# TJUMMG/OCPG

Hardware: AMD Instinct MI355X
Metric: clips/sec fwd+bwd (5x384x640, R101) (higher is better)
Workload: dtype bf16

## Files before the change

include/ocpg_hip.h:

```cpp
#ifndef OCPG_HIP_H
#define OCPG_HIP_H
#include <stdint.h>

#ifdef __cplusplus
extern "C" {
#endif

int ocpg_msda_fwd_f32(const float* value, const int64_t* shapes, const int64_t* level_start,
                      const float* loc, const float* attn,
                      int N, int S, int M, int D, int L, int Lq, int P,
                      float* out, const int64_t* shapes_host, void* stream);
int ocpg_msda_fwd_f64(const double* value, const int64_t* shapes, const int64_t* level_start,
                      const double* loc, const double* attn,
                      int N, int S, int M, int D, int L, int Lq, int P,
                      double* out, void* stream);

int ocpg_msda_bwd_f32(const float* value, const int64_t* shapes, const int64_t* level_start,
                      const float* loc, const float* attn, const float* grad_out,
                      int N, int S, int M, int D, int L, int Lq, int P,
                      float* grad_value, float* grad_loc, float* grad_attn,
                      const int64_t* shapes_host, void* stream);
int ocpg_msda_bwd_value_f32(const float* loc, const float* attn, const float* grad_out,
                            int N, int S, int M, int D, int L, int Lq, int P,
                            float* grad_value, const int64_t* shapes_host, void* stream);
// ... 37 lines not shown
                      int N, int S, int M, int D, int L, int Lq, int P,
                      float* grad_value, float* grad_loc, float* grad_attn,
                      const int64_t* shapes_host, int* sel_state, int dtype, void* stream);
int ocpg_msda_bwd_value_h16(const float* loc, const float* attn, const void* grad_out,
                            int N, int S, int M, int D, int L, int Lq, int P,
                            float* grad_value, const int64_t* shapes_host, int* sel_state, int dtype, void* stream);
int ocpg_msda_bwd_locattn_h16(const void* value, const int64_t* shapes, const int64_t* level_start,
                              const float* loc, const float* attn, const void* grad_out,
                              int N, int S, int M, int D, int L, int Lq, int P,
                              float* grad_loc, float* grad_attn, int dtype, void* stream);
int ocpg_msda_fused_fwd_h16(const void* value, const int64_t* shapes, const int64_t* level_start,
                            const float* qproj, const float* ref,
                            int N, int S, int M, int D, int L, int Lq, int P,
                            void* out, float* loc_out, float* attn_out, int dtype, void* stream);
int ocpg_msda_fused_bwd_qproj_h16(const void* value, const int64_t* shapes, const int64_t* level_start,
                                  const float* loc, const float* attn, const void* grad_out,
                                  int N, int S, int M, int D, int L, int Lq, int P,
                                  float* grad_qproj, int dtype, void* stream);

int ocpg_bn_act_fwd(const void* x, const float* scale, const float* shift, const void* skip, void* y,
                    long long n_outer, int C, long long inner, int relu, int dtype, void* stream);
int ocpg_bn_act_bwd(const void* gy, const void* y, const float* scale, void* gx, void* gskip,
                    long long n_outer, int C, long long inner, int relu, int dtype, void* stream);

int ocpg_gemm_dgrad_bn_tile(long long M, int N, int K);
int ocpg_gemm_dgrad_bn(const void* a, const void* w, const void* c, const void* mask, const float* scale, void* out, void* out_skip,
                       long long M, int N, int K, int dtype, int tile, void* stream);

int ocpg_gemm_dgrad_mask(const void* a, const void* w, const void* mask, float scale, void* out, float* colsum_part, long long M, int N,
                         int K, int dtype, int tile, void* stream);
int ocpg_gemm_bias_relu_dropout_fwd(const void* x, const void* w, const void* bias, float p, unsigned long long seed,
                                    unsigned long long offset, const unsigned long long* rng_base, void* h, long long M, int N, int K,
                                    int dtype, int tile, int round_gemm, void* stream);

int ocpg_win_attn_fwd(const void* qkv, const float* biasT, const int* region, float scale, int BW, int NW, int N, int H,
                      int head_dim, void* out, float* lse, int dtype, void* stream);
int ocpg_win_attn_bwd(const void* qkv, const float* bias, const float* biasT, const int* region, float scale, int BW, int NW,
                      int N, int H, int head_dim, const void* out, const void* dout, const float* lse, void* dqkv, float* Dbuf,
                      float* dbiasT, int dtype, void* stream);

int ocpg_win_attn_bwd_mfma(const void* qkv, const float* bias, const float* biasT, const int* region, float scale, int BW, int NW, int N,
                           int H, int head_dim, const void* out, const void* dout, const float* lse, void* dqkv, float* Dbuf, void* dS,
                           int dtype, void* stream);

int ocpg_win_attn_dtable_supported(int N, int head_dim, int dtype, int T);
int ocpg_win_attn_bwd_mfma_dtable(const void* qkv, const float* bias, const float* biasT, const int* region, float scale, int BW, int NW,
                                  int N, int H, int head_dim, const void* out, const void* dout, const float* lse, void* dqkv, float* Dbuf,
                                  const int* tok_code, int code_off, int T, float* partials, float* dtable, int dtype, void* stream);

int ocpg_dynmask_fwd_f32(const float* feats, const float* params, const float* refpix, int BT, int Q, int C, int H, int W,
                         int stride, float* out, float* pre1, void* stream);

int ocpg_dynmask_bwd_pre_f32(const float* dout, const float* pre1, const float* params, int BT, int Q, int C, int H, int W,
                             int stride, float* dpre, float* part, float* w0d, void* stream);
int ocpg_dynmask_bwd_fin_f32(const float* part, const float* params, const float* refpix, const float* dw0, int BT, int Q, int C,
                             int H, int W, float* dparams, float* dref, void* stream);

int ocpg_im2col3x3_nhwc(const void* x, int N, int H, int W, int C, int stride, int dil, void* cols, int dtype, void* stream);
int ocpg_col2im3x3_nhwc(const void* dcols, int N, int H, int W, int C, int stride, int dil, void* dx, int dtype, void* stream);

int ocpg_conv3x3_mfma_fwd(const void* x, const void* w, const float* scale, const float* bias, int relu, int N, int H, int W,
                          int Cin, int Cout, int stride, void* y, void* stream);
int ocpg_conv3x3_mfma_fwd_cols(const void* x, const void* w, const float* scale, const float* bias, int relu, int N, int H, int W, int Cin,
                               int Cout, int stride, void* y, void* cols, void* stream);
int ocpg_conv3x3_mfma_dgrad(const void* dy, const void* wT, int N, int H, int W, int Cin, int Cout, int stride, void* dx,
                            void* stream);
int ocpg_conv3x3_mfma_dgrad_masked(const void* dy, const void* wT, const void* mask_y, const float* scale, int N, int H, int W, int Cin,
                                   int Cout, int stride, void* dx, void* stream);
int ocpg_conv3x3_mfma_dgrad_w(const void* dy, const void* w, const void* mask_y, const float* scale, int N, int H, int W, int Cin, int Cout,
                              int stride, void* dx, void* stream);
int ocpg_conv3x3_mfma_body_splits(long long M, int ncols, int kchannels);
int ocpg_conv3x3_mfma_fwd_bn_splitk(const void* x, const void* w, const float* scale, const float* shift, int relu, int N, int H, int W, int Cin,
                                    int Cout, int stride, int splits, float* part, void* y, void* stream);
int ocpg_conv3x3_mfma_dgrad_w_splitk(const void* dy, const void* w, const void* mask_y, const float* scale, int N, int H, int W, int Cin,
                                     int Cout, int stride, int splits, float* part, void* dx, void* stream);
int ocpg_conv3x3_mfma_wgrad_splits(int N, int H, int W, int Cin, int Cout, int stride);
int ocpg_conv3x3_mfma_wgrad(const void* gz, const void* x, int N, int H, int W, int Cin, int Cout, int stride, void* part, void* stream);
int ocpg_conv3x3_mfma_fwd_cols_h16(const void* x, const void* w, const float* scale, const float* bias, int relu, int N, int H, int W, int Cin,
                                   int Cout, int stride, void* y, void* cols, int dtype, void* stream);
int ocpg_conv3x3_mfma_dgrad_w_h16(const void* dy, const void* w, const void* mask_y, const float* scale, int N, int H, int W, int Cin, int Cout,
                                  int stride, void* dx, int dtype, void* stream);
int ocpg_conv3x3_mfma_wgrad_h16(const void* gz, const void* x, int N, int H, int W, int Cin, int Cout, int stride, void* part, int dtype,
                                void* stream);
int ocpg_conv3x3_mfma_dgrad_w_s2(const void* dy, const void* w, const void* mask_y, const float* scale, int N, int H, int W, int Cin, int Cout,
                                 int stride, void* dx, void* stream);
int ocpg_conv3x3_mfma_dgrad_w_s2_h16(const void* dy, const void* w, const void* mask_y, const float* scale, int N, int H, int W, int Cin, int Cout,
                                     int stride, void* dx, int dtype, void* stream);

int ocpg_conv3x3_mfma_splits(int N, int H, int W, int Cin, int Cout, int stride);
int ocpg_conv3x3_mfma_fwd_splitk(const void* x, const void* w, const float* bias, int N, int H, int W, int Cin, int Cout, int stride,
                                 int splits, float* part, void* y, int out_dt, void* cols, void* stream);
int ocpg_conv3x3_mfma_fwd_splitk_h16(const void* x, const void* w, const float* bias, int N, int H, int W, int Cin, int Cout, int stride,
                                     int splits, float* part, void* y, int out_dt, void* cols, int dtype, void* stream);

int ocpg_gemm(const void* A, const void* B, void* C, const void* bias, int dtype, int out_dtype, int transA, int transB,
              long long M, long long N, long long K, long long lda, long long ldb, long long ldc, long long batch,
              long long strideA, long long strideB, long long strideC, float alpha, float beta, void* stream);
long long ocpg_gemm_plans(void);
long long ocpg_gemm_tuned(long long* changed);
long long ocpg_gemm_tune_rejected(void);
void ocpg_gemm_set_tuning(int on);
long long ocpg_gemm_export_picks(long long* buf, long long cap_pairs);
int ocpg_gemm_import_picks(const long long* buf, long long n_pairs);
int ocpg_gemm_bn_act(const void* A, const void* W, void* D, const float* scale, const float* shift, const void* skip, int relu, int dtype,
                     long long M, long long N, long long K, void* stream);

int ocpg_levelset_fwd_f32(const float* x, const float* feats, const float* box, int Lr, int N, int C, int CF, int h, int w, float* sums,
                          float* coef, float* loss, void* stream);
int ocpg_levelset_bwd_f32(const float* x, const float* feats, const float* box, const float* coef, const float* gloss, int Lr, int N,
                          int C, int CF, int h, int w, float* gx, float* gfeat, void* stream);
int ocpg_proj_fwd_f32(const float* x, const float* tcmax, const float* trmax, const float* tcmean, const float* trmean, int Lr, int B,
                      int T, int H, int W, float* colstat, float* rowstat, float* IU, float* loss, void* stream);
int ocpg_proj_bwd_f32(const float* x, const float* tcmax, const float* trmax, const float* tcmean, const float* trmean,
                      const float* colstat, const float* rowstat, const float* IU, const float* gloss, int Lr, int B, int T, int H, int W,
                      float* Gc, float* Gr, float* gx, void* stream);

int ocpg_matcher_cost_f32(const float* logits, const float* boxes, const float* masks, long long sl, long long sb, long long st,
                          long long sq, const float* gt, const float* tboxes, const float* valid, const long long* labels, int Lr,
                          int B, int T, int Q, int K, int h, int w, float wc, float wb, float wg, float wm, float wd, float* sums,
                          float* cost, int* bad, void* stream);

int ocpg_dropout_add_ln_fwd(const void* x, const float* res, const float* gamma, const float* beta, long long R, int C, float eps, float p,
                            unsigned long long seed, unsigned long long offset, const unsigned long long* rng_base, int x_dtype, float* y,
                            float* mean, float* rstd, void* stream);
int ocpg_dropout_add_ln_bwd(const float* gy, const void* x, const float* res, const float* gamma, const float* mean, const float* rstd,
                            long long R, int C, float p, unsigned long long seed, unsigned long long offset, const unsigned long long* rng_base,
                            int x_dtype, void* gx, float* gres, float* dgb_part, void* stream);
long long ocpg_dropout_add_ln_bwd_slots(long long R);
int ocpg_dropout_add_ln_fwd_ex(const void* x, const float* res, const float* gamma, const float* beta, long long R, int C, float eps, float p,
                               unsigned long long seed, unsigned long long offset, const unsigned long long* rng_base, int x_dtype, float* y,
                               float* mean, float* rstd, const float* addend, float* y_add, void* y_lp, int lp_dtype, void* stream);
int ocpg_dropout_add_ln_bwd_ex(const void* g0, int g0_dtype, const void* g1, int g1_dtype, const void* g2, int g2_dtype, const void* x,
                               const float* res, const float* gamma, const float* mean, const float* rstd, long long R, int C, float p,
                               unsigned long long seed, unsigned long long offset, const unsigned long long* rng_base, int x_dtype, void* gx,
                               float* gres, float* dgb_part, float* gxsum_part, void* stream);
int ocpg_bias_relu_dropout_fwd(const void* a, const void* bias, long long R, int C, float p, unsigned long long seed,
                               unsigned long long offset, const unsigned long long* rng_base, int dtype, void* h, void* stream);
int ocpg_bias_relu_dropout_bwd(const void* gh, const void* h, long long R, int C, float p, int dtype, void* ga, float* dbias_part,
                               void* stream);
long long ocpg_bias_relu_dropout_bwd_slots(long long R, int C, int dtype);

int ocpg_multi_cast(const long long* srcs, const long long* dsts, const long long* numels, const long long* chunk_prefix, int n,
                    long long total_chunks, int src_dtype, int dst_dtype, void* stream);
int ocpg_multi_cast_sum(const long long* srcs, const long long* dsts, const long long* numels, const long long* chunk_prefix,
                        const long long* splits, const long long* strides, int n, long long total_chunks, int src_dtype, int dst_dtype,
                        void* stream);
long long ocpg_colsum_blocks(long long R);
int ocpg_colsum_partials(const void* x, long long R, int C, int dtype, float* part, void* stream);

int ocpg_grad_norm_clip(const long long* grads, const long long* numels, const long long* chunk_prefix, int n, long long total_chunks,
                        float max_norm, float* partials, float* norm_and_coef, void* stream);
int ocpg_adamw_step(const long long* params, const long long* grads, const long long* exp_avg, const long long* exp_avg_sq,
                    const long long* numels, const long long* chunk_prefix, const float* lr, const float* weight_decay, int n,
                    long long total_chunks, const float* norm_and_coef, double beta1, double beta2, double eps, long long step, void* stream);
int ocpg_grad_norm_clip_amp(const long long* grads, const long long* numels, const long long* chunk_prefix, int n, long long total_chunks,
                            float max_norm, float* partials, const float* grad_scale, const float* found_inf, double beta1, double beta2,
                            float* amp_state, void* stream);
int ocpg_adamw_step_amp(const long long* params, const long long* grads, const long long* exp_avg, const long long* exp_avg_sq,
                        const long long* numels, const long long* chunk_prefix, const float* lr, const float* weight_decay, int n,
                        long long total_chunks, const float* amp_state, double beta1, double beta2, double eps, void* stream);

int ocpg_det_loss_fwd_f32(const float* logits, const float* boxes, const long long* src, const float* valid, const long long* labels,
                          const float* tboxes, const float* num_boxes, float alpha, int Lr, int B, int T, int Q, int K, float* loss, int* bad,
                          void* stream);
int ocpg_det_loss_bwd_f32(const float* logits, const float* boxes, const long long* src, const float* valid, const long long* labels,
                          const float* tboxes, const float* num_boxes, const float* gloss, float alpha, int Lr, int B, int T, int Q, int K,
// ... 158 lines not shown
```

ocpg_amd/_lib.py:

```python
import ctypes
import glob
import os
import re

import torch

_HERE = os.path.dirname(os.path.abspath(__file__))
LIB_PATH = os.environ.get("OCPG_HIP_LIB") or os.path.join(_HERE, "lib", "libocpg_hip.so")
_lib = None

DTYPE_CODE = {torch.float32: 0, torch.bfloat16: 1, torch.float16: 2}
H16_CODE = {torch.bfloat16: 1, torch.float16: 2}

_BY_VALUE = {"int": ctypes.c_int, "long long": ctypes.c_longlong, "unsigned long long": ctypes.c_ulonglong, "float": ctypes.c_float,
             "double": ctypes.c_double}
_RETURNS = {"int": ctypes.c_int, "long long": ctypes.c_longlong, "void": None, "const char*": ctypes.c_char_p}
_DECL = re.compile(r"([\w\s*]+?)\b(\w+)\s*\(([^()]*)\)")


def _declarations(text):
    text = re.sub(r"/\*.*?\*/", " ", text, flags=re.S)
    if "//" in text:
        raise ValueError("a // comment in the header: the signature parser reads block comments only")
    text = re.sub(r"^[ \t]*#.*$", "", text, flags=re.M)
    text = re.sub(r'extern\s+"C"\s*\{', "", text)
    text = re.sub(r"^[ \t]*\}[ \t]*$", "", text, flags=re.M)

    def norm(t):
        return re.sub(r"\s*\*\s*", "*", " ".join(t.split()))
    out = []
    for stmt in text.split(";"):
        if not stmt.strip():
            continue
        m = _DECL.fullmatch(stmt.strip())
        if m is None:
            raise ValueError(f"not a function declaration: {' '.join(stmt.split())!r}")
        params = []
        for p in m.group(3).split(","):
            if p.strip() in ("", "void"):
                continue
            t, pname = re.fullmatch(r"(.*?)(\w*)", p.strip(), flags=re.S).groups()
            params.append((norm(t), pname))
        out.append((norm(m.group(1)), m.group(2), params))
    return out


def parse_header(text):
    out = {}
    for ret, name, params in _declarations(text):
        if ret not in _RETURNS:
            raise ValueError(f"{name}: return type {ret!r} is not one of {sorted(_RETURNS)}")
        argtypes = []
        for t, pname in params:
            if "*" not in t and t not in _BY_VALUE:
                raise ValueError(f"{name}: parameter {pname!r} has by-value type {t!r}, not one of {sorted(_BY_VALUE)}")
            argtypes.append(ctypes.c_void_p if "*" in t else _BY_VALUE[t])
        out[name] = (_RETURNS[ret], argtypes)
    return out


_HEADERS = "".join(open(h).read() for h in sorted(glob.glob(os.path.join(os.path.dirname(_HERE), "include", "*.h"))))
_PARSED = parse_header(_HEADERS)
SIGNATURES = {name: argtypes for name, (_, argtypes) in _PARSED.items() if name != "ocpg_hip_version"}


_TIMING = {"on": False, "events": []}
_UNTIMED = frozenset(name for _, name, params in _declarations(_HEADERS)
                     if name in SIGNATURES and ("void*", "stream") not in params)


def enable_kernel_timing(on=True):
    _TIMING["on"] = on
    _TIMING["events"] = []


def collect_kernel_timing(work=None):
    torch.cuda.synchronize()
    out = {}
    for name, args, e0, e1 in _TIMING["events"]:
        d = out.setdefault(name, {"ms": 0.0, "n": 0, "work": 0.0, "modelled": 0})
        d["ms"] += e0.elapsed_time(e1)
        d["n"] += 1
        w = work(name, args) if work is not None else None
        if isinstance(w, tuple):
            d["work_lowp"] = d.get("work_lowp", 0.0) + (w[0] if w[1] else 0.0)
            w = w[0]
        if w is not None:
            d["work"] += w
            d["modelled"] += 1
    _TIMING["events"] = []
    _TIMING["on"] = False
    return out


CENSUS = {"on": False, "calls": {}}
CENSUS_ALSO = {"ocpg_conv3x3_mfma_dgrad_w_s2": "ocpg_conv3x3_mfma_dgrad_w", "ocpg_conv3x3_mfma_dgrad_w_s2_h16": "ocpg_conv3x3_mfma_dgrad_w_h16",
               "ocpg_dropout_add_ln_fwd_ex": "ocpg_dropout_add_ln_fwd", "ocpg_dropout_add_ln_bwd_ex": "ocpg_dropout_add_ln_bwd"}


def census(on=True):
    CENSUS["on"] = on
    if on:
        CENSUS["calls"] = {}
    return CENSUS["calls"]


class _Lib:

    def __init__(self, cdll):
        self._cdll = cdll

    def __getattr__(self, name):
        fn = getattr(self._cdll, name)
        if name not in SIGNATURES or name in _UNTIMED:
            setattr(self, name, fn)
            return fn
        timed = not name.startswith("ocpg_msda_")

        def call(*a):
            if CENSUS["on"]:
                rc = fn(*a)
                if rc == 0:
                    for k in (name, CENSUS_ALSO.get(name)):
                        if k is not None:
                            CENSUS["calls"][k] = CENSUS["calls"].get(k, 0) + 1
                return rc
            if not (timed and _TIMING["on"]):
                return fn(*a)
            e0, e1 = torch.cuda.Event(enable_timing=True), torch.cuda.Event(enable_timing=True)
            e0.record()
            rc = fn(*a)
            e1.record()
            _TIMING["events"].append((name, tuple(getattr(x, "value", x) for x in a), e0, e1))
            return rc
        setattr(self, name, call)
        return call


def lib():
    global _lib
    if _lib is None:
        if not os.path.exists(LIB_PATH):
            raise RuntimeError(
                f"{LIB_PATH} not found: build it with `python -m ocpg_amd.csrc.build` "
                "(hipcc --offload-arch=gfx950). The HIP extension is mandatory; there is no CPU/PyTorch fallback.")
        L = ctypes.CDLL(LIB_PATH)
        for name, (restype, argtypes) in _PARSED.items():
            fn = getattr(L, name)
            fn.argtypes = argtypes
            fn.restype = restype
        _lib = _Lib(L)
    return _lib


def check(status, what):
    if status != 0:
        if status <= -1000:
            raise RuntimeError(f"{what}: invalid argument #{-status - 1000}")
        raise RuntimeError(f"{what}: HIP error {-status}")


def stream_ptr():
    return ctypes.c_void_p(torch.cuda.current_stream().cuda_stream)


def require_gpu(name, t):
    if not t.is_cuda:
        raise RuntimeError(f"{name} must be a GPU tensor: Not implemented on the CPU")
    if not t.is_contiguous():
        raise RuntimeError(f"{name} tensor has to be contiguous")
```

ocpg_amd/csrc/conv3x3_wgrad.hip:

```cpp
#include <hip/hip_bf16.h>
#include <hip/hip_fp16.h>
#include <hip/hip_runtime.h>
#include <stdint.h>

#include <cstdlib>

#include "../../include/ocpg_hip.h"
#include "h16_elem.h"

namespace {

typedef ocpg_h16::h16x8 bf16x8;
typedef short s4 __attribute__((ext_vector_type(4)));
typedef ocpg_h16::f32x16 f32x16;
using ocpg_h16::Bf16;
using ocpg_h16::Fp16;

constexpr int NT = 256, TM = 64, TN = 64, LROW = 72;

__device__ __forceinline__ bf16x8 tr_frag(const short* tile, int r0, int pitch, int c0, int lane) {
  const int li = lane & 15, grp = lane >> 4, fh = lane >> 5;
  const short* p = tile + (r0 + (8 * fh + (li >> 2)) * pitch) * LROW + c0 + 16 * (grp & 1) + 4 * (li & 3);
  const s4 lo = __builtin_amdgcn_ds_read_tr16_b64_v4i16((__attribute__((address_space(3))) s4*)p);
  const s4 hi = __builtin_amdgcn_ds_read_tr16_b64_v4i16((__attribute__((address_space(3))) s4*)(p + 4 * pitch * LROW));
  bf16x8 r;
  r[0] = lo[0]; r[1] = lo[1]; r[2] = lo[2]; r[3] = lo[3]; r[4] = hi[0]; r[5] = hi[1]; r[6] = hi[2]; r[7] = hi[3];
  return r;
}

__device__ __forceinline__ uint4 keep(uint4 v, bool yes) { return make_uint4(yes ? v.x : 0u, yes ? v.y : 0u, yes ? v.z : 0u, yes ? v.w : 0u); }

struct WG {
  int N, H, W, Ho, Wo, Cin, Cout, stride, seg, xw, rows_per_split;
};

#define WGRAD_KERNEL conv3x3_wgrad
#define WGRAD_ELEM Bf16
#include "conv3x3_wgrad_kernel.h"
#undef WGRAD_KERNEL
#undef WGRAD_ELEM
#define WGRAD_KERNEL conv3x3_wgrad_f16
#define WGRAD_ELEM Fp16
#include "conv3x3_wgrad_kernel.h"
#undef WGRAD_KERNEL
#undef WGRAD_ELEM

inline int seg_of(int stride) { return stride == 1 ? 64 : 32; }

}

extern "C" {

int ocpg_conv3x3_mfma_wgrad_splits(int N, int H, int W, int Cin, int Cout, int stride) {
  if (N <= 0 || H <= 0 || W <= 0 || Cin <= 0 || Cout <= 0 || (stride != 1 && stride != 2)) return 0;
  const long long rows = (long long)N * ((H - 1) / stride + 1);
  const long long tiles = (long long)((Cout + TM - 1) / TM) * ((Cin + TN - 1) / TN);
  static const int target = [] { const char* e = std::getenv("OCPG_WGRAD_WGS"); return e && *e ? std::atoi(e) : 256; }();
  long long s = (target + tiles - 1) / tiles;
  if (s > rows) s = rows;
  if (s < 1) s = 1;
  const long long rps = (rows + s - 1) / s;
  return (int)((rows + rps - 1) / rps);
}

int ocpg_conv3x3_mfma_wgrad_h16(const void* gz, const void* x, int N, int H, int W, int Cin, int Cout, int stride, void* part, int dtype,
                                void* stream) {
  if (dtype != 1 && dtype != 2) return -1010;
  if (N < 0 || H <= 0 || W <= 0 || Cin <= 0 || Cout <= 0) return -1003;
  if ((stride != 1 && stride != 2) || Cin % 8 != 0 || Cout % 8 != 0) return -2000;
  if (N == 0) return 0;
  if (!gz) return -1001;
  if (!x) return -1002;
  if (!part) return -1009;
  WG g;
  g.N = N; g.H = H; g.W = W; g.Ho = (H - 1) / stride + 1; g.Wo = (W - 1) / stride + 1; g.Cin = Cin; g.Cout = Cout; g.stride = stride;
  g.seg = seg_of(stride);
  g.xw = (g.seg - 1) * stride + 3;
  const int splits = ocpg_conv3x3_mfma_wgrad_splits(N, H, W, Cin, Cout, stride);
  const long long rows = (long long)N * g.Ho;
  g.rows_per_split = (int)((rows + splits - 1) / splits);
  const dim3 grid((unsigned)((Cout + TM - 1) / TM), (unsigned)((Cin + TN - 1) / TN), (unsigned)splits);
  if (dtype == 2) {
    if (stride == 1) conv3x3_wgrad_f16<1, 64><<<grid, NT, 0, (hipStream_t)stream>>>((const __half*)gz, (const __half*)x, g, (__half*)part);
    else conv3x3_wgrad_f16<2, 32><<<grid, NT, 0, (hipStream_t)stream>>>((const __half*)gz, (const __half*)x, g, (__half*)part);
  } else if (stride == 1) {
    conv3x3_wgrad<1, 64><<<grid, NT, 0, (hipStream_t)stream>>>((const __hip_bfloat16*)gz, (const __hip_bfloat16*)x, g, (__hip_bfloat16*)part);
  } else {
    conv3x3_wgrad<2, 32><<<grid, NT, 0, (hipStream_t)stream>>>((const __hip_bfloat16*)gz, (const __hip_bfloat16*)x, g, (__hip_bfloat16*)part);
  }
  const hipError_t e = hipGetLastError();
  return e == hipSuccess ? 0 : -(int)e;
}

int ocpg_conv3x3_mfma_wgrad(const void* gz, const void* x, int N, int H, int W, int Cin, int Cout, int stride, void* part, void* stream) {
  return ocpg_conv3x3_mfma_wgrad_h16(gz, x, N, H, W, Cin, Cout, stride, part, 1, stream);
}

}
```

ocpg_amd/models/ops/functions/conv_bn_func.py:

```python
import os

import torch
from torch.autograd import Function
from torch.autograd.function import once_differentiable

from ...._lib import DTYPE_CODE as _DT, H16_CODE, check, lib

_H16 = H16_CODE.keys()
_CL = torch.channels_last
EPILOGUE = os.environ.get("OCPG_GEMM_EPILOGUE", "1") != "0"
FWD_COLS = os.environ.get("OCPG_CONV3X3_FWD_COLS", "0") != "0"
SKIP_GRAD_IN_GEMM = os.environ.get("OCPG_SKIP_GRAD_IN_GEMM", "1") != "0"
_SKIP_TOKENS = {}
PREMASK = os.environ.get("OCPG_PREMASK_DGRAD", "1") != "0"
_PREMASK_TOKENS = {}
FUSED_DGRAD_BN = os.environ.get("OCPG_FUSED_DGRAD_BN", "1") != "0"
_DGRAD_BN_DECLINED = (-2000, -2001, -2002)


def reset_skip_tokens():
    _SKIP_TOKENS.clear()
    _PREMASK_TOKENS.clear()


# ... 221 lines not shown
    return x.shape[1] >= 256 and (x.shape[1] * x.element_size()) % 16 == 0 and rows <= 12288


class Conv3x3BNAct(Function):
    @staticmethod
    def forward(ctx, x, w, scale, shift, relu, stride, dil, splits):
        n, c, h, wd = x.shape
        co = w.shape[0]
        ho, wo = (h - 1) // stride + 1, (wd - 1) // stride + 1
        m = n * ho * wo
        dt = _DT[x.dtype]
        L = lib()
        st = torch.cuda.current_stream().cuda_stream
        cols = torch.empty((m, 9 * c), dtype=x.dtype, device=x.device)
        check(L.ocpg_im2col3x3_nhwc(x.data_ptr(), n, h, wd, c, stride, dil, cols.data_ptr(), dt, st), "ocpg_im2col3x3_nhwc")
        w2 = w.permute(0, 2, 3, 1).reshape(co, 9 * c)
        if not w2.is_contiguous():
            w2 = w2.contiguous()
        y = torch.empty((n, co, ho, wo), dtype=x.dtype, device=x.device, memory_format=_CL)
        rc = L.ocpg_gemm_bn_act(cols.data_ptr(), w2.data_ptr(), y.data_ptr(), scale.data_ptr(), shift.data_ptr(), None, int(relu), dt, m, co,
                                9 * c, st) if EPILOGUE else -1105
        if rc and rc != -1105:
            check(rc, "ocpg_gemm_bn_act")
        if rc:
            check(L.ocpg_gemm(cols.data_ptr(), w2.data_ptr(), y.data_ptr(), None, dt, dt, 0, 1, m, co, 9 * c, 9 * c, 9 * c, co, 1, 0, 0, 0, 1.0,
                              0.0, st), "ocpg_gemm")
            check(L.ocpg_bn_act_fwd(y.data_ptr(), scale.data_ptr(), shift.data_ptr(), None, y.data_ptr(), m, co, 1, int(relu), dt, st),
                  "ocpg_bn_act_fwd")
        ctx.save_for_backward(cols, w2, y, scale)
        ctx.meta = (bool(relu), splits, (n, c, h, wd, ho, wo, stride, dil), w.shape)
        return y

    @staticmethod
    @once_differentiable
    def backward(ctx, gy):
        cols, w2, y, scale = ctx.saved_tensors
        relu, splits, (n, c, h, wd, ho, wo, stride, dil), wshape = ctx.meta
        co = w2.shape[0]
        m, k = cols.shape
        dt = _DT[y.dtype]
        L = lib()
        st = torch.cuda.current_stream().cuda_stream
        if gy.dtype != y.dtype or not gy.is_contiguous(memory_format=_CL):
            gy = gy.to(y.dtype).contiguous(memory_format=_CL)
        gz = torch.empty_like(y)
        check(L.ocpg_bn_act_bwd(gy.data_ptr(), y.data_ptr(), scale.data_ptr(), gz.data_ptr(), None, m, co, 1, int(relu), dt, st), "ocpg_bn_act_bwd")
        gx = gw = None
        if ctx.needs_input_grad[0]:
            dcols = torch.empty((m, k), dtype=y.dtype, device=y.device)
            check(L.ocpg_gemm(gz.data_ptr(), w2.data_ptr(), dcols.data_ptr(), None, dt, dt, 0, 0, m, k, co, co, k, k, 1, 0, 0, 0, 1.0, 0.0, st),
                  "ocpg_gemm")
            gx = torch.empty((n, c, h, wd), dtype=y.dtype, device=y.device, memory_format=_CL)
            check(L.ocpg_col2im3x3_nhwc(dcols.data_ptr(), n, h, wd, c, stride, dil, gx.data_ptr(), dt, st), "ocpg_col2im3x3_nhwc")
        if ctx.needs_input_grad[1]:
            if splits > 1 and m % splits == 0:
                r = m // splits
                part = torch.empty((splits, co, k), dtype=y.dtype, device=y.device)
                check(L.ocpg_gemm(gz.data_ptr(), cols.data_ptr(), part.data_ptr(), None, dt, dt, 1, 0, co, k, r, co, k, k, splits, r * co, r * k,
                                  co * k, 1.0, 0.0, st), "ocpg_gemm")
                g2 = part.sum(0)
            else:
                g2 = torch.empty((co, k), dtype=y.dtype, device=y.device)
                check(L.ocpg_gemm(gz.data_ptr(), cols.data_ptr(), g2.data_ptr(), None, dt, dt, 1, 0, co, k, m, co, k, k, 1, 0, 0, 0, 1.0, 0.0, st),
                      "ocpg_gemm")
            gw = g2.view(co, 3, 3, c).permute(0, 3, 1, 2)
        return gx, gw, None, None, None, None, None, None


def conv3x3_bn_act(x, w, scale, shift, relu, stride, dil, splits):
    return Conv3x3BNAct.apply(x, w, scale, shift, relu, int(stride), int(dil), splits)


def eligible3x3_mfma(x, conv):
    if x.dtype == torch.float16 and (BODY_SPLITK or not DGRAD_OWN_WEIGHT):
        return False
    return (x.is_cuda and x.dim() == 4 and x.dtype in _H16 and conv.kernel_size == (3, 3) and conv.groups == 1
            and conv.bias is None and conv.stride[0] == conv.stride[1] and conv.stride[0] in (1, 2) and conv.dilation == (1, 1)
            and conv.padding == (1, 1) and conv.padding_mode == "zeros" and x.is_contiguous(memory_format=_CL)
            and x.shape[1] % 64 == 0 and conv.out_channels % 64 == 0 and x.shape[1] >= _MFMA_MIN_C and conv.out_channels >= _MFMA_MIN_C)


BODY_SPLITK = os.environ.get("OCPG_CONV3X3_SPLITK", "0") != "0"
WGRAD_OWN = os.environ.get("OCPG_WGRAD_OWN", "1") != "0"
DGRAD_OWN_WEIGHT = os.environ.get("OCPG_DGRAD_OWN_WEIGHT", "1") != "0"
DGRAD_S2_CLASSES = os.environ.get("OCPG_DGRAD_S2_CLASSES", "1") != "0"
_MFMA_MIN_C = int(os.environ.get("OCPG_MFMA_CONV3X3_MIN_C", "128"))


class Conv3x3MfmaBNAct(Function):

    @staticmethod
    def forward(ctx, x, w, scale, shift, relu, stride, splits):
        n, c, h, wd = x.shape
        co = w.shape[0]
        ho, wo = (h - 1) // stride + 1, (wd - 1) // stride + 1
        if not _both16(x, w):
            raise RuntimeError(f"Conv3x3MfmaBNAct: x and w must share one 16-bit dtype, got {x.dtype} and {w.dtype}")
        fp16 = x.dtype == torch.float16
        if fp16 and (BODY_SPLITK or not DGRAD_OWN_WEIGHT):
            raise RuntimeError("Conv3x3MfmaBNAct: OCPG_CONV3X3_SPLITK / OCPG_DGRAD_OWN_WEIGHT=0 select kernels that have no fp16 form")
        w2 = w.permute(0, 2, 3, 1)
        if not w2.is_contiguous():
            w2 = w2.contiguous()
        y = torch.empty((n, co, ho, wo), dtype=x.dtype, device=x.device, memory_format=_CL)
        st = torch.cuda.current_stream().cuda_stream
        cols = torch.empty((n * ho * wo, 9 * c), dtype=x.dtype, device=x.device) if (FWD_COLS and ctx.needs_input_grad[1]) else None
        sp = int(lib().ocpg_conv3x3_mfma_body_splits(n * ho * wo, co, c)) if (BODY_SPLITK and cols is None) else 1
        if sp > 1:
            part = torch.empty((sp, n * ho * wo, co), dtype=torch.float32, device=x.device)
            check(lib().ocpg_conv3x3_mfma_fwd_bn_splitk(x.data_ptr(), w2.data_ptr(), scale.data_ptr(), shift.data_ptr(), int(relu), n, h, wd, c, co, stride,
                                                        sp, part.data_ptr(), y.data_ptr(), st), "ocpg_conv3x3_mfma_fwd_bn_splitk")
        elif fp16:
            check(lib().ocpg_conv3x3_mfma_fwd_cols_h16(x.data_ptr(), w2.data_ptr(), scale.data_ptr(), shift.data_ptr(), int(relu), n, h, wd, c, co,
                                                       stride, y.data_ptr(), None if cols is None else cols.data_ptr(), 2, st),
                  "ocpg_conv3x3_mfma_fwd_cols_h16")
        else:
            check(lib().ocpg_conv3x3_mfma_fwd_cols(x.data_ptr(), w2.data_ptr(), scale.data_ptr(), shift.data_ptr(), int(relu), n, h, wd, c, co, stride,
                                                   y.data_ptr(), None if cols is None else cols.data_ptr(), st), "ocpg_conv3x3_mfma_fwd_cols")
        ctx.has_cols = cols is not None
        if cols is not None:
            ctx.save_for_backward(x, w2, y, scale, cols)
        else:
            ctx.save_for_backward(x, w2, y, scale)
        from ...amp_cache import is_cast_copy
        ctx.meta = (bool(relu), splits, stride)
        ctx.w_cast = is_cast_copy(w)
        tok = _claim_token(x) if PREMASK else None
        ctx.premask = tok if (tok is not None and not tok["skip"] and ctx.needs_input_grad[0]) else None
        ctx.offer = (_offer_token(y, scale, False, "OCPG_FUSED_DGRAD_BN")
                     if (FUSED_DGRAD_BN and relu and any(ctx.needs_input_grad)) else None)
        return y

    @staticmethod
    @once_differentiable
    def backward(ctx, gy):
        x, w2, y, scale = ctx.saved_tensors[:4]
        relu, splits, stride = ctx.meta
        n, c, h, wd = x.shape
        co, ho, wo = y.shape[1], y.shape[2], y.shape[3]
        m, k = n * ho * wo, 9 * c
        dt = _DT[y.dtype]
        fp16 = dt == 2
        L = lib()
        st = torch.cuda.current_stream().cuda_stream
        if gy.dtype != y.dtype or not gy.is_contiguous(memory_format=_CL):
            gy = gy.to(y.dtype).contiguous(memory_format=_CL)
        fused = _take_token(ctx.offer, gy)
        if fused is not None:
            gz = gy
        else:
            gz = torch.empty_like(y)
            check(L.ocpg_bn_act_bwd(gy.data_ptr(), y.data_ptr(), scale.data_ptr(), gz.data_ptr(), None, m, co, 1, int(relu), dt, st), "ocpg_bn_act_bwd")
        gx = gw = None
        if ctx.needs_input_grad[0]:
            gx = torch.empty((n, c, h, wd), dtype=y.dtype, device=y.device, memory_format=_CL)
            tok = ctx.premask
            mask_ptr, scale_ptr = (x.data_ptr(), tok["scale"].data_ptr()) if tok is not None else (None, None)
            sp = int(L.ocpg_conv3x3_mfma_body_splits(n * h * wd, c, co)) if (BODY_SPLITK and DGRAD_OWN_WEIGHT and c % 8 == 0 and not fp16) else 1
            s2 = stride == 2 and DGRAD_S2_CLASSES
            if fp16:
                fn = L.ocpg_conv3x3_mfma_dgrad_w_s2_h16 if s2 else L.ocpg_conv3x3_mfma_dgrad_w_h16
                check(fn(gz.data_ptr(), w2.data_ptr(), mask_ptr, scale_ptr, n, h, wd, c, co, stride, gx.data_ptr(), 2, st),
                      "ocpg_conv3x3_mfma_dgrad_w_s2_h16" if s2 else "ocpg_conv3x3_mfma_dgrad_w_h16")
            elif sp > 1:
                part = torch.empty((sp, n * h * wd, c), dtype=torch.float32, device=y.device)
                check(L.ocpg_conv3x3_mfma_dgrad_w_splitk(gz.data_ptr(), w2.data_ptr(), mask_ptr, scale_ptr, n, h, wd, c, co, stride, sp, part.data_ptr(),
                                                         gx.data_ptr(), st), "ocpg_conv3x3_mfma_dgrad_w_splitk")
            elif DGRAD_OWN_WEIGHT and c % 8 == 0:
                fn = L.ocpg_conv3x3_mfma_dgrad_w_s2 if s2 else L.ocpg_conv3x3_mfma_dgrad_w
                check(fn(gz.data_ptr(), w2.data_ptr(), mask_ptr, scale_ptr, n, h, wd, c, co, stride, gx.data_ptr(), st),
                      "ocpg_conv3x3_mfma_dgrad_w_s2" if s2 else "ocpg_conv3x3_mfma_dgrad_w")
            else:
                wt = w2.permute(3, 1, 2, 0).contiguous()
                check(L.ocpg_conv3x3_mfma_dgrad_masked(gz.data_ptr(), wt.data_ptr(), mask_ptr, scale_ptr, n, h, wd, c, co, stride, gx.data_ptr(), st),
                      "ocpg_conv3x3_mfma_dgrad_masked")
            if tok is not None:
                _fill_token(tok, gx)
        if ctx.needs_input_grad[1]:
            from ...amp_cache import side_wgrad
            with side_wgrad(ctx.w_cast, gz, x) as sw:
                st = torch.cuda.current_stream().cuda_stream
                if WGRAD_OWN and not ctx.has_cols and c % 8 == 0 and co % 8 == 0:
                    sp = int(L.ocpg_conv3x3_mfma_wgrad_splits(n, h, wd, c, co, stride))
                    part = torch.empty((sp, co, k), dtype=y.dtype, device=y.device)
                    if fp16:
                        check(L.ocpg_conv3x3_mfma_wgrad_h16(gz.data_ptr(), x.data_ptr(), n, h, wd, c, co, stride, part.data_ptr(), 2, st),
                              "ocpg_conv3x3_mfma_wgrad_h16")
                    else:
                        check(L.ocpg_conv3x3_mfma_wgrad(gz.data_ptr(), x.data_ptr(), n, h, wd, c, co, stride, part.data_ptr(), st), "ocpg_conv3x3_mfma_wgrad")
                    g2 = _reduce_partials(part, ctx.w_cast) if sp > 1 else part[0]
                else:
                    if ctx.has_cols:
                        cols = ctx.saved_tensors[4]
                    else:
                        cols = torch.empty((m, k), dtype=y.dtype, device=y.device)
                        check(L.ocpg_im2col3x3_nhwc(x.data_ptr(), n, h, wd, c, stride, 1, cols.data_ptr(), dt, st), "ocpg_im2col3x3_nhwc")
                    if splits > 1 and m % splits == 0:
                        r = m // splits
                        part = torch.empty((splits, co, k), dtype=y.dtype, device=y.device)
                        check(L.ocpg_gemm(gz.data_ptr(), cols.data_ptr(), part.data_ptr(), None, dt, dt, 1, 0, co, k, r, co, k, k, splits, r * co, r * k,
                                          co * k, 1.0, 0.0, st), "ocpg_gemm")
                        g2 = _reduce_partials(part, ctx.w_cast)
                    else:
                        g2 = torch.empty((co, k), dtype=y.dtype, device=y.device)
                        check(L.ocpg_gemm(gz.data_ptr(), cols.data_ptr(), g2.data_ptr(), None, dt, dt, 1, 0, co, k, m, co, k, k, 1, 0, 0, 0, 1.0, 0.0, st),
                              "ocpg_gemm")
                gw = sw.publish(g2).view(co, 3, 3, c).permute(0, 3, 1, 2)
        return gx, gw, None, None, None, None, None


def conv3x3_mfma_bn_act(x, w, scale, shift, relu, stride, splits):
    return Conv3x3MfmaBNAct.apply(x, w, scale, shift, relu, int(stride), splits)


def eligible3x3_splitk(x, conv):
    if not (x.is_cuda and x.dim() == 4 and x.dtype in _H16 and conv.kernel_size == (3, 3) and conv.groups == 1
            and conv.stride[0] == conv.stride[1] and conv.stride[0] in (1, 2) and conv.dilation == (1, 1) and conv.padding == (1, 1)
            and conv.padding_mode == "zeros" and x.is_contiguous(memory_format=_CL) and x.shape[1] % 64 == 0 and conv.out_channels % 64 == 0):
        return False
    n, c, h, w = x.shape
    return int(lib().ocpg_conv3x3_mfma_splits(n, h, w, c, conv.out_channels, conv.stride[0])) > 1


class Conv3x3SplitK(Function):

    @staticmethod
    def forward(ctx, x, w, b, stride):
        n, c, h, wd = x.shape
        co = w.shape[0]
        ho, wo = (h - 1) // stride + 1, (wd - 1) // stride + 1
        m = n * ho * wo
        L = lib()
        st = torch.cuda.current_stream().cuda_stream
        w2 = w.permute(0, 2, 3, 1)
        if not w2.is_contiguous():
            w2 = w2.contiguous()
        if not _both16(x, w):
            raise RuntimeError(f"Conv3x3SplitK: x and w must share one 16-bit dtype, got {x.dtype} and {w.dtype}")
        splits = int(L.ocpg_conv3x3_mfma_splits(n, h, wd, c, co, stride))
        part = torch.empty((splits, m, co), dtype=torch.float32, device=x.device)
        y = torch.empty((n, co, ho, wo), dtype=x.dtype, device=x.device, memory_format=_CL)
        need_w = ctx.needs_input_grad[1]
        cols = torch.empty((m, 9 * c), dtype=x.dtype, device=x.device) if need_w else None
        bf = None if b is None else b.float()
        if x.dtype == torch.float16:
            check(L.ocpg_conv3x3_mfma_fwd_splitk_h16(x.data_ptr(), w2.data_ptr(), None if bf is None else bf.data_ptr(), n, h, wd, c, co, stride, splits,
                                                     part.data_ptr(), y.data_ptr(), 2, None if cols is None else cols.data_ptr(), 2, st),
                  "ocpg_conv3x3_mfma_fwd_splitk_h16")
        else:
            check(L.ocpg_conv3x3_mfma_fwd_splitk(x.data_ptr(), w2.data_ptr(), None if bf is None else bf.data_ptr(), n, h, wd, c, co, stride, splits,
                                                 part.data_ptr(), y.data_ptr(), 1, None if cols is None else cols.data_ptr(), st),
                  "ocpg_conv3x3_mfma_fwd_splitk")
        ctx.save_for_backward(w2, cols if need_w else w2)
        ctx.meta = (n, c, h, wd, ho, wo, stride, b is not None, need_w)
        return y

    @staticmethod
    @once_differentiable
    def backward(ctx, gy):
        w2, cols = ctx.saved_tensors
        n, c, h, wd, ho, wo, stride, has_b, need_w = ctx.meta
        co = w2.shape[0]
        m, k = n * ho * wo, 9 * c
        L = lib()
        st = torch.cuda.current_stream().cuda_stream
        dt = _DT[w2.dtype]
        if gy.dtype != w2.dtype or not gy.is_contiguous(memory_format=_CL):
            gy = gy.to(w2.dtype).contiguous(memory_format=_CL)
# ... 23 lines not shown
```

Measured before the change: 68.03.

## Add ring-buffered 3x3 conv weight-gradient kernel reusing input rows across output rows

Adds a new wgrad kernel that streams output-gradient rows through double-buffered LDS and keeps a ring of input rows. Each loaded input row is reused by all three vertical taps instead of being re-read per row. Global loads are prefetched several steps ahead in registers, and the 9 taps are split between two wave groups running at different priorities. It is enabled by default for eligible shapes and falls back to the old kernel when shapes are rejected, at the cost of higher register and LDS use and a more complex indexing scheme.

```diff
diff --git a/include/ocpg_hip.h b/include/ocpg_hip.h
--- a/include/ocpg_hip.h
+++ b/include/ocpg_hip.h
@@ -143,6 +143,9 @@
                                   int stride, void* dx, int dtype, void* stream);
 int ocpg_conv3x3_mfma_wgrad_h16(const void* gz, const void* x, int N, int H, int W, int Cin, int Cout, int stride, void* part, int dtype,
                                 void* stream);
+int ocpg_conv3x3_mfma_wgrad_ring(const void* gz, const void* x, int N, int H, int W, int Cin, int Cout, int stride, void* part, void* stream);
+int ocpg_conv3x3_mfma_wgrad_ring_h16(const void* gz, const void* x, int N, int H, int W, int Cin, int Cout, int stride, void* part, int dtype,
+                                     void* stream);
 int ocpg_conv3x3_mfma_dgrad_w_s2(const void* dy, const void* w, const void* mask_y, const float* scale, int N, int H, int W, int Cin, int Cout,
                                  int stride, void* dx, void* stream);
 int ocpg_conv3x3_mfma_dgrad_w_s2_h16(const void* dy, const void* w, const void* mask_y, const float* scale, int N, int H, int W, int Cin, int Cout,
diff --git a/ocpg_amd/_lib.py b/ocpg_amd/_lib.py
--- a/ocpg_amd/_lib.py
+++ b/ocpg_amd/_lib.py
@@ -95,6 +95,7 @@
 
 CENSUS = {"on": False, "calls": {}}
 CENSUS_ALSO = {"ocpg_conv3x3_mfma_dgrad_w_s2": "ocpg_conv3x3_mfma_dgrad_w", "ocpg_conv3x3_mfma_dgrad_w_s2_h16": "ocpg_conv3x3_mfma_dgrad_w_h16",
+               "ocpg_conv3x3_mfma_wgrad_ring": "ocpg_conv3x3_mfma_wgrad", "ocpg_conv3x3_mfma_wgrad_ring_h16": "ocpg_conv3x3_mfma_wgrad_h16",
                "ocpg_dropout_add_ln_fwd_ex": "ocpg_dropout_add_ln_fwd", "ocpg_dropout_add_ln_bwd_ex": "ocpg_dropout_add_ln_bwd"}
 
 
diff --git a/ocpg_amd/csrc/conv3x3_wgrad.hip b/ocpg_amd/csrc/conv3x3_wgrad.hip
--- a/ocpg_amd/csrc/conv3x3_wgrad.hip
+++ b/ocpg_amd/csrc/conv3x3_wgrad.hip
@@ -46,6 +46,21 @@
 #undef WGRAD_ELEM
 
 inline int seg_of(int stride) { return stride == 1 ? 64 : 32; }
+
+constexpr int NTR = 512;
+template <int V>
+struct IC { static constexpr int value = V; };
+
+#define WGRAD_RING_KERNEL conv3x3_wgrad_ring
+#define WGRAD_ELEM Bf16
+#include "conv3x3_wgrad_ring_kernel.h"
+#undef WGRAD_RING_KERNEL
+#undef WGRAD_ELEM
+#define WGRAD_RING_KERNEL conv3x3_wgrad_ring_f16
+#define WGRAD_ELEM Fp16
+#include "conv3x3_wgrad_ring_kernel.h"
+#undef WGRAD_RING_KERNEL
+#undef WGRAD_ELEM
 
 }
 
@@ -96,4 +111,42 @@
   return ocpg_conv3x3_mfma_wgrad_h16(gz, x, N, H, W, Cin, Cout, stride, part, 1, stream);
 }
 
+int ocpg_conv3x3_mfma_wgrad_ring_h16(const void* gz, const void* x, int N, int H, int W, int Cin, int Cout, int stride, void* part, int dtype,
+                                     void* stream) {
+  if (dtype != 1 && dtype != 2) return -1010;
+  if (N < 0 || H <= 0 || W <= 0 || Cin <= 0 || Cout <= 0) return -1003;
+  if ((stride != 1 && stride != 2) || Cin % 8 != 0 || Cout % 8 != 0) return -2000;
+  if ((W - 1) / stride + 1 > seg_of(stride)) return -2000;
+  if ((long long)W * Cin > 0x7fffffffLL || (long long)W * Cout > 0x7fffffffLL) return -2000;
+  if (N == 0) return 0;
+  if (!gz) return -1001;
+  if (!x) return -1002;
+  if (!part) return -1009;
+  WG g;
+  g.N = N; g.H = H; g.W = W; g.Ho = (H - 1) / stride + 1; g.Wo = (W - 1) / stride + 1; g.Cin = Cin; g.Cout = Cout; g.stride = stride;
+  g.seg = seg_of(stride);
+  g.xw = (g.seg - 1) * stride + 3;
+  const int splits = ocpg_conv3x3_mfma_wgrad_splits(N, H, W, Cin, Cout, stride);
+  const long long rows = (long long)N * g.Ho;
+  g.rows_per_split = (int)((rows + splits - 1) / splits);
+  const dim3 grid((unsigned)((Cout + TM - 1) / TM), (unsigned)((Cin + TN - 1) / TN), (unsigned)splits);
+  const hipStream_t st = (hipStream_t)stream;
+  const int ks = (g.Wo + 15) / 16;
+#define RING(S_, SEG_, KS_)                                                                                                  \
+  if (dtype == 2) conv3x3_wgrad_ring_f16<S_, SEG_, KS_><<<grid, NTR, 0, st>>>((const __half*)gz, (const __half*)x, g, (__half*)part); \
+  else conv3x3_wgrad_ring<S_, SEG_, KS_><<<grid, NTR, 0, st>>>((const __hip_bfloat16*)gz, (const __hip_bfloat16*)x, g, (__hip_bfloat16*)part)
+  if (stride == 1) {
+    if (ks == 1) { RING(1, 64, 1); } else if (ks == 2) { RING(1, 64, 2); } else if (ks == 3) { RING(1, 64, 3); } else { RING(1, 64, 4); }
+  } else {
+    if (ks == 1) { RING(2, 32, 1); } else { RING(2, 32, 2); }
+  }
+#undef RING
+  const hipError_t e = hipGetLastError();
+  return e == hipSuccess ? 0 : -(int)e;
 }
+
+int ocpg_conv3x3_mfma_wgrad_ring(const void* gz, const void* x, int N, int H, int W, int Cin, int Cout, int stride, void* part, void* stream) {
+  return ocpg_conv3x3_mfma_wgrad_ring_h16(gz, x, N, H, W, Cin, Cout, stride, part, 1, stream);
+}
+
+}
diff --git a/ocpg_amd/csrc/conv3x3_wgrad_ring_kernel.h b/ocpg_amd/csrc/conv3x3_wgrad_ring_kernel.h
--- /dev/null
+++ b/ocpg_amd/csrc/conv3x3_wgrad_ring_kernel.h
@@ -0,0 +1,152 @@
+template <int S, int SEG, int KS>
+__global__ __launch_bounds__(NTR) void WGRAD_RING_KERNEL(const WGRAD_ELEM::T* __restrict__ gz, const WGRAD_ELEM::T* __restrict__ x, WG g,
+                                                         WGRAD_ELEM::T* __restrict__ part) {
+  using E = WGRAD_ELEM;
+  using T = E::T;
+  constexpr int XW = (SEG - 1) * S + 3;
+  constexpr int R = 3 + S, P = 3 - S;
+  constexpr int XL = (S * XW * 8 + NTR - 1) / NTR;
+  constexpr int NST = S == 1 ? 4 : 3;
+  constexpr int GSZ = SEG * LROW, SLOT = XW * LROW;
+  __shared__ __attribute__((aligned(16))) short lds[2 * GSZ + R * SLOT];
+  short* const Gs = lds;
+  short* const Xs = lds + 2 * GSZ;
+  const int tid = threadIdx.x, lane = tid & 63, wave = __builtin_amdgcn_readfirstlane(tid >> 6);
+  const int grp = wave >> 2, wm = wave & 1, wn = (wave >> 1) & 1;
+  const int co0 = blockIdx.x * TM, ci0 = blockIdx.y * TN;
+  const long long rows = (long long)g.N * g.Ho;
+  const long long r_lo = (long long)blockIdx.z * g.rows_per_split, r_hi = min(rows, r_lo + g.rows_per_split);
+  constexpr int kp = KS * 16;
+  const long long r0c = min(r_lo, rows - 1);
+  const int n0 = (int)(r0c / g.Ho), y0 = (int)(r0c - (long long)n0 * g.Ho);
+  const int nsteps = r_hi > r_lo ? (int)(r_hi - r_lo) + P * (1 + (int)((r_hi - 1) / g.Ho) - n0) : 0;
+  f32x16 acc[5];
+#pragma unroll
+  for (int t = 0; t < 5; ++t)
+#pragma unroll
+    for (int r = 0; r < 16; ++r) acc[t][r] = 0.f;
+  struct Regs { uint4 rg, rx[XL]; unsigned zr; };
+  Regs RA, RB, RC, RD;
+  int goff, gl, xoff[XL], xl[XL];
+  unsigned zc = 0, rsel = 0;
+  {
+    const int e = tid & (SEG * 8 - 1), k = e >> 3, sg = e & 7;
+    zc |= (k < g.Wo && co0 + sg * 8 + 8 <= g.Cout) ? 0u : 1u;
+    goff = min(k, g.Wo - 1) * g.Cout + min(co0 + sg * 8, g.Cout - 8);
+    gl = k * LROW + sg * 8;
+  }
+#pragma unroll
+  for (int i = 0; i < XL; ++i) {
+    int e = tid + i * NTR;
+    if (e >= S * XW * 8) e -= NTR;
+    const int sg = e & 7, j = (e >> 3) % XW, r = (e >> 3) / XW, xi = j - 1;
+    zc |= (xi >= 0 && xi < g.W && ci0 + sg * 8 + 8 <= g.Cin) ? 0u : 2u << i;
+    rsel |= r ? 1u << i : 0u;
+    xoff[i] = min(max(xi, 0), g.W - 1) * g.Cin + min(ci0 + sg * 8, g.Cin - 8);
+    xl[i] = j * LROW + sg * 8;
+  }
+  int fn = n0, fy = y0 - P;
+  auto fetch = [&](Regs& R_) __attribute__((always_inline)) {
+    R_.rg = *reinterpret_cast<const uint4*>(gz + ((long long)fn * g.Ho + max(fy, 0)) * g.Wo * g.Cout + goff);
+    const int y_0 = fy * S + 2 - S, y_1 = y_0 + S - 1;
+    const int c_0 = min(max(y_0, 0), g.H - 1), c_1 = min(max(y_1, 0), g.H - 1);
+    const T* row0 = x + ((long long)fn * g.H + c_0) * g.W * g.Cin;
+    const int drow = (c_1 - c_0) * g.W * g.Cin;
+#pragma unroll
+    for (int i = 0; i < XL; ++i) R_.rx[i] = *reinterpret_cast<const uint4*>(row0 + (xoff[i] + (((rsel >> i) & 1u) ? drow : 0)));
+    R_.zr = ((y_0 < 0 || y_0 >= g.H) ? 1u : 0u) | ((y_1 < 0 || y_1 >= g.H) ? 2u : 0u);
+    if (fy < 0 || (long long)fn * g.Ho + fy + 1 < r_hi) {
+      if (++fy == g.Ho) { fy = -P; ++fn; }
+    }
+  };
+  int pb = 0, ps = 0;
+  auto park = [&](const Regs& R_) __attribute__((always_inline)) {
+    *reinterpret_cast<uint4*>(Gs + pb * GSZ + gl) = keep(R_.rg, !(zc & 1u));
+    const int s_0 = ps * SLOT, s_1 = (ps + 1 >= R ? ps + 1 - R : ps + 1) * SLOT;
+#pragma unroll
+    for (int i = 0; i < XL; ++i) {
+      const bool second = S == 2 && ((rsel >> i) & 1u);
+      const bool zero = ((zc >> (1 + i)) & 1u) || ((R_.zr >> (second ? 1 : 0)) & 1u);
+      *reinterpret_cast<uint4*>(Xs + (second ? s_1 : s_0) + xl[i]) = keep(R_.rx[i], !zero);
+    }
+    pb ^= 1;
+    ps += S;
+    if (ps >= R) ps -= R;
+  };
+  int cb = 0, cs = 0, cy = y0, ph = P;
+  auto mult = [&](auto first, auto count) __attribute__((always_inline)) {
+    constexpr int T0 = decltype(first)::value, NTAP = decltype(count)::value;
+    int row[3];
+#pragma unroll
+    for (int ky = 0; ky < 3; ++ky) {
+      int s = cs + ky + S - 3;
+      if (s < 0) s += R;
+      if (s >= R) s -= R;
+      row[ky] = s * SLOT;
+    }
+#pragma unroll
+    for (int k0 = 0; k0 < kp; k0 += 16) {
+      const bf16x8 a = tr_frag(Gs + cb * GSZ, k0, 1, wm * 32, lane);
+#pragma unroll
+      for (int t = 0; t < NTAP; ++t) {
+        const int ky = (T0 + t) / 3, kx = (T0 + t) - ky * 3;
+        const bf16x8 b = tr_frag(Xs + row[ky], k0 * S + kx, S, wn * 32, lane);
+        acc[t] = E::mfma(a, b, acc[t]);
+      }
+    }
+  };
+  auto step = [&](Regs& R_) __attribute__((always_inline)) {
+#ifndef WG_CUT_LOAD
+    park(R_);
+    fetch(R_);
+#endif
+#ifndef WG_CUT_COMPUTE
+    if (ph == 0) {
+      if (grp == 0) mult(IC<0>{}, IC<5>{});
+      else mult(IC<5>{}, IC<4>{});
+    }
+#endif
+    cb ^= 1;
+    cs += S;
+    if (cs >= R) cs -= R;
+    if (ph > 0) --ph;
+    else if (++cy == g.Ho) { cy = 0; ph = P; }
+    __syncthreads();
+  };
+  if (grp) __builtin_amdgcn_s_setprio(1);
+  fetch(RA); fetch(RB);
+  if constexpr (NST >= 3) fetch(RC);
+  if constexpr (NST == 4) fetch(RD);
+#ifndef WG_CUT_LOAD
+  park(RA);
+  fetch(RA);
+#endif
+  __syncthreads();
+  if (nsteps > 0)
+    for (int c = 0;;) {
+      step(RB);
+      if (++c >= nsteps) break;
+      if constexpr (NST >= 3) {
+        step(RC);
+        if (++c >= nsteps) break;
+      }
+      if constexpr (NST == 4) {
+        step(RD);
+        if (++c >= nsteps) break;
+      }
+      step(RA);
+      if (++c >= nsteps) break;
+    }
+  const int ci = ci0 + wn * 32 + (lane & 31);
+  if (ci < g.Cin) {
+    T* out = part + (long long)blockIdx.z * g.Cout * 9 * g.Cin;
+#pragma unroll
+    for (int t = 0; t < 5; ++t)
+#pragma unroll
+      for (int r = 0; r < 16; ++r) {
+        const int co = co0 + wm * 32 + (r & 3) + 8 * (r >> 2) + 4 * (lane >> 5);
+        const int tap = grp * 5 + t;
+        if (tap < 9 && co < g.Cout) out[((long long)co * 9 + tap) * g.Cin + ci] = E::narrow(acc[t][r]);
+      }
+  }
+}
diff --git a/ocpg_amd/models/ops/functions/conv_bn_func.py b/ocpg_amd/models/ops/functions/conv_bn_func.py
--- a/ocpg_amd/models/ops/functions/conv_bn_func.py
+++ b/ocpg_amd/models/ops/functions/conv_bn_func.py
@@ -327,6 +327,7 @@
 
 BODY_SPLITK = os.environ.get("OCPG_CONV3X3_SPLITK", "0") != "0"
 WGRAD_OWN = os.environ.get("OCPG_WGRAD_OWN", "1") != "0"
+WGRAD_RING = os.environ.get("OCPG_WGRAD_RING", "1") != "0"
 DGRAD_OWN_WEIGHT = os.environ.get("OCPG_DGRAD_OWN_WEIGHT", "1") != "0"
 DGRAD_S2_CLASSES = os.environ.get("OCPG_DGRAD_S2_CLASSES", "1") != "0"
 _MFMA_MIN_C = int(os.environ.get("OCPG_MFMA_CONV3X3_MIN_C", "128"))
@@ -428,7 +429,14 @@
                 if WGRAD_OWN and not ctx.has_cols and c % 8 == 0 and co % 8 == 0:
                     sp = int(L.ocpg_conv3x3_mfma_wgrad_splits(n, h, wd, c, co, stride))
                     part = torch.empty((sp, co, k), dtype=y.dtype, device=y.device)
-                    if fp16:
+                    rc = -2000
+                    if WGRAD_RING and fp16:
+                        rc = L.ocpg_conv3x3_mfma_wgrad_ring_h16(gz.data_ptr(), x.data_ptr(), n, h, wd, c, co, stride, part.data_ptr(), 2, st)
+                    elif WGRAD_RING:
+                        rc = L.ocpg_conv3x3_mfma_wgrad_ring(gz.data_ptr(), x.data_ptr(), n, h, wd, c, co, stride, part.data_ptr(), st)
+                    if rc != -2000:
+                        check(rc, "ocpg_conv3x3_mfma_wgrad_ring_h16" if fp16 else "ocpg_conv3x3_mfma_wgrad_ring")
+                    elif fp16:
                         check(L.ocpg_conv3x3_mfma_wgrad_h16(gz.data_ptr(), x.data_ptr(), n, h, wd, c, co, stride, part.data_ptr(), 2, st),
                               "ocpg_conv3x3_mfma_wgrad_h16")
                     else:
```

New measurement: 68.94, median of 6. 1.3% higher.
